# technosaurus/PDMP3

Hardware: AMD Instinct MI355X
Metric: MP3 frames/sec (44.1 kHz stereo 320 kbps), transforms-only hot path (higher is better)
Workload: dtype f32; 1 GPU; C2 (BASELINE configs[1]): 2048 stereo frames = 4096 granules per GPU per step, pre-Huffman-decoded spectra resident in HBM, one stream; frames_per_gpu=2048, granules_per_gpu=4096, seed=0x5eed0000c2, chunk_frames=auto

## Files before the change

pdmp3_amd/csrc/decode_core.h:

```cpp
#pragma once

#include <math.h>
#include <stdint.h>
#include <string.h>
#include "../../include/pdmp3_hip.h"

namespace pdmp3 {
struct ConstBank;
}

#if defined(__HIPCC__)
#define PD_FN __device__ __forceinline__
#define PD_SLOW_FN __device__ __attribute__((noinline))
#define PD_MFN __device__ __forceinline__
#define PD_HD __host__ __device__ __forceinline__
#define PD_FMA(a, b, c) __builtin_fmaf((a), (b), (c))
#define PD_CLOCK() __builtin_amdgcn_s_memtime()
#define PD_UNROLL _Pragma("unroll")
#define PD_UNROLL_N(n) _Pragma(PD_STR_(unroll n))
#define PD_STR_(x) #x
#define PD_NOUNROLL _Pragma("nounroll")
#define PD_SCHED_FENCE() __builtin_amdgcn_sched_barrier(0)
#define PD_PIN(x) asm volatile("" : "+v"(x))
#define PD_ANY(c) (__builtin_amdgcn_ballot_w64(c) != 0ull)
#define PD_LANE() ((int)(threadIdx.x & 63))
#define PD_UNIFORM(x) __builtin_amdgcn_readfirstlane((int)(x))
#define PD_SHFL_XOR(v, m) __shfl_xor((v), (m))
#define PD_WAVE_SYNC()                                       \
  __builtin_amdgcn_fence(__ATOMIC_RELEASE, "wavefront");    \
  __builtin_amdgcn_wave_barrier();                          \
  __builtin_amdgcn_fence(__ATOMIC_ACQUIRE, "wavefront")
#define PD_STORE_DEVICE(p, v) __hip_atomic_store((p), (v), __ATOMIC_RELAXED, __HIP_MEMORY_SCOPE_AGENT)
#define PD_LOAD_DEVICE(p) __hip_atomic_load((p), __ATOMIC_RELAXED, __HIP_MEMORY_SCOPE_AGENT)
#define PD_VMEM_DRAIN() asm volatile("s_waitcnt vmcnt(0)" ::: "memory")
#define PD_SLEEP() __builtin_amdgcn_s_sleep(4)
#define PD_SETPRIO(x) __builtin_amdgcn_s_setprio(x)
#define PD_LDS_FLAG(p) (*(volatile __attribute__((address_space(3))) unsigned*)(p))
#define PD_BALLOT(c) ((unsigned long long)__builtin_amdgcn_ballot_w64(c))
namespace pdmp3 {
typedef const __attribute__((address_space(4))) ConstBank* BankPtr;
}
#define PD_LAUNDER(p) asm volatile("" : "+s"(p))
#define PD_UNIFORM_PTR(T, p) ((T)(((unsigned long long)(unsigned)PD_UNIFORM((int)((unsigned long long)(p) >> 32)) << 32) | (unsigned)PD_UNIFORM((int)(unsigned long long)(p))))
#define PD_UNCHECKED_INDEX(v, lo, n) (v)
#define PD_FMED3(x, lo, hi) __builtin_amdgcn_fmed3f((x), (lo), (hi))
namespace pdmp3 {
typedef float f32x2 __attribute__((ext_vector_type(2)));
typedef unsigned short u16x2 __attribute__((ext_vector_type(2)));
typedef float f32x4 __attribute__((ext_vector_type(4)));
__device__ __forceinline__ f32x2 fma2(f32x2 a, f32x2 b, f32x2 c) { return __builtin_elementwise_fma(a, b, c); }
__device__ __forceinline__ f32x4 mfma16(float a, float b, f32x4 c) { return __builtin_amdgcn_mfma_f32_16x16x4f32(a, b, c, 0, 0, 0); }
__device__ __forceinline__ void permlane32_swap(int& a, int& b) {
  const auto r = __builtin_amdgcn_permlane32_swap((unsigned)a, (unsigned)b, false, false);
  a = (int)r[0];
  b = (int)r[1];
}
__device__ __forceinline__ void mul9_rtz_32767(const float* x, float* p) {
#define PD_M(n, m) "v_mul_f32 %" #n ", 0x46fffe00, %" #m "\n\t"
  asm volatile(
      "s_setreg_imm32_b32 hwreg(HW_REG_MODE, 0, 2), 3\n\t"
      "s_nop 1\n\t"
      PD_M(0, 9) PD_M(1, 10) PD_M(2, 11) PD_M(3, 12) PD_M(4, 13) PD_M(5, 14) PD_M(6, 15) PD_M(7, 16) PD_M(8, 17)
      "s_setreg_imm32_b32 hwreg(HW_REG_MODE, 0, 2), 0\n\t"
      "s_nop 1"
      : "=&v"(p[0]), "=&v"(p[1]), "=&v"(p[2]), "=&v"(p[3]), "=&v"(p[4]), "=&v"(p[5]), "=&v"(p[6]), "=&v"(p[7]), "=&v"(p[8])
      : "v"(x[0]), "v"(x[1]), "v"(x[2]), "v"(x[3]), "v"(x[4]), "v"(x[5]), "v"(x[6]), "v"(x[7]), "v"(x[8]));
#undef PD_M
}
__device__ __forceinline__ void mul18_rtz_32767(const float* x, float* p) {
  mul9_rtz_32767(x, p);
  mul9_rtz_32767(x + 9, p + 9);
}
}
#else
namespace pdmp3 {
namespace emu {
int lane();
void wave_sync();
void wave_yield();
float shfl_xor(float v, int mask);
bool any(bool c);
unsigned long long ballot(bool c);
void mfma16(float a, float b, float* cd);
void permlane32_swap(int* a, int* b);
}
}
#define PD_FN static inline
#define PD_SLOW_FN static
#define PD_MFN inline
#define PD_HD static inline
#define PD_FMA(a, b, c) __builtin_fmaf((a), (b), (c))
#define PD_CLOCK() 0ull
#define PD_UNROLL
#define PD_UNROLL_N(n)
#define PD_NOUNROLL
#define PD_SCHED_FENCE() ((void)0)
#define PD_PIN(x) ((void)0)
#define PD_ANY(c) (::pdmp3::emu::any(c))
#define PD_LANE() (::pdmp3::emu::lane())
#define PD_UNIFORM(x) ((int)(x))
#define PD_SHFL_XOR(v, m) (::pdmp3::emu::shfl_xor((v), (m)))
#define PD_WAVE_SYNC() ::pdmp3::emu::wave_sync()
#define PD_STORE_DEVICE(p, v) (*(p) = (v))
#define PD_LOAD_DEVICE(p) (*(p))
#define PD_VMEM_DRAIN() ::pdmp3::emu::wave_sync()
#define PD_SLEEP() ::pdmp3::emu::wave_yield()
#define PD_SETPRIO(x) ((void)0)
#define PD_LDS_FLAG(p) (*(volatile unsigned*)(p))
#define PD_BALLOT(c) (::pdmp3::emu::ballot(c))
namespace pdmp3 {
typedef const ConstBank* BankPtr;
}
#define PD_LAUNDER(p) ((void)0)
#define PD_UNIFORM_PTR(T, p) (p)
#define PD_UNCHECKED_INDEX(v, lo, n) ((unsigned)((v) - (lo)) < (unsigned)(n) ? (v) : 0)
namespace pdmp3 {
typedef float f32x2 __attribute__((vector_size(8)));
typedef unsigned short u16x2 __attribute__((vector_size(4)));
typedef float f32x4 __attribute__((vector_size(16)));
static inline f32x2 fma2(f32x2 a, f32x2 b, f32x2 c) { return (f32x2){__builtin_fmaf(a[0], b[0], c[0]), __builtin_fmaf(a[1], b[1], c[1])}; }
static inline f32x4 mfma16(float a, float b, f32x4 c) {
  float cd[4] = {c[0], c[1], c[2], c[3]};
  emu::mfma16(a, b, cd);
  return (f32x4){cd[0], cd[1], cd[2], cd[3]};
}
static inline void permlane32_swap(int& a, int& b) { emu::permlane32_swap(&a, &b); }
static inline float pd_fmed3_host(float x, float lo, float hi) {
  if (x != x) return lo < hi ? lo : hi;
  return x < lo ? lo : (x > hi ? hi : x);
}
static inline void mul18_rtz_32767(const float* x, float* p) {
  for (int t = 0; t < 18; t++) {
    const double d = (double)x[t] * 32767.0;
    float f = (float)d;
    if (f == f && !__builtin_isinf(f) && __builtin_fabs((double)f) > __builtin_fabs(d)) f = __builtin_nextafterf(f, 0.0f);
    else if (__builtin_isinf(f) && !__builtin_isinf(x[t])) f = __builtin_copysignf(0x1.fffffep+127f, f);
    p[t] = f;
  }
}
}
#define PD_FMED3(x, lo, hi) (::pdmp3::pd_fmed3_host((x), (lo), (hi)))
#endif

#ifndef PD_EXP_SKIP
#define PD_EXP_SKIP 0
#endif
#ifndef PD_C36_MQ
#define PD_C36_MQ 1
#endif
#ifndef PD_CHUNK_FAST_REQUANT
#define PD_CHUNK_FAST_REQUANT 0
#endif
#ifndef PD_PRIO_MFMA
#define PD_PRIO_MFMA 2
#endif
#ifndef PD_PRIO_WINDOW
#define PD_PRIO_WINDOW 0
#endif
#ifndef PD_PRIO_REQUANT
#define PD_PRIO_REQUANT 1
#endif
// ... 99 lines not shown
  int nch, sfreq, mode, mode_ext;
  int ver;
  int lsf_scale;
  int iso;
  int count1_0, count1_1, flags0, flags1;
  PD_MFN int flags(int ch) const { return ch ? flags1 : flags0; }
  PD_MFN bool is_short(int ch) const {
    const int f = flags(ch);
    return (f & PDMP3_GC_WIN_SWITCH) && ((f & PDMP3_GC_BLOCK_TYPE_MASK) >> PDMP3_GC_BLOCK_TYPE_SHIFT) == 2;
  }
  PD_MFN bool is_mixed(int ch) const { return (flags(ch) & PDMP3_GC_MIXED) != 0; }
  PD_MFN int block_type(int ch) const { return (flags(ch) & PDMP3_GC_BLOCK_TYPE_MASK) >> PDMP3_GC_BLOCK_TYPE_SHIFT; }
  PD_MFN int kind(int ch) const { return is_short(ch) ? (is_mixed(ch) ? 2 : 1) : 0; }
};

template <bool RARE = true>
PD_FN GranuleInfo granule_info(const WaveData& L) {
  GranuleInfo g;
  const uint32_t w0 = (uint32_t)PD_UNIFORM(*reinterpret_cast<const uint32_t*>(&L.side[0][0]));
  const uint32_t w1 = (uint32_t)PD_UNIFORM(*reinterpret_cast<const uint32_t*>(&L.side[1][0]));
  const int fr = PD_UNIFORM(L.side[0][7]);
  g.fr = fr;
  g.iso = PD_UNIFORM(L.side[0][offsetof(pdmp3_gc_side, iso)]);
  g.sfreq = fr & PDMP3_FR_SFREQ_MASK;
  if (g.sfreq > 2) g.sfreq = 2;
  g.ver = 0;
  g.lsf_scale = 0;
  if (RARE) {
    const int lsf0 = PD_UNIFORM(L.side[0][offsetof(pdmp3_gc_side, lsf)]);
    g.ver = lsf0 & PDMP3_LSF_VERSION_MASK;
    if (g.ver > 2) g.ver = 2;
  }
  if (RARE && g.ver) {
    g.sfreq += 3 * g.ver;
    g.iso |= PDMP3_GC_ISO_MS_ALL | PDMP3_GC_ISO_IS_SHORT | PDMP3_GC_ISO_IS_STD;
    g.lsf_scale = (PD_UNIFORM(L.side[1][offsetof(pdmp3_gc_side, lsf)]) & PDMP3_LSF_IS_SCALE) ? 1 : 0;
  }
  g.mode = (fr & PDMP3_FR_MODE_MASK) >> PDMP3_FR_MODE_SHIFT;
  g.mode_ext = (fr & PDMP3_FR_MODEEXT_MASK) >> PDMP3_FR_MODEEXT_SHIFT;
  g.nch = (g.mode == 3) ? 1 : 2;
  g.count1_0 = (int)(w0 & 0xffffu);
  g.count1_1 = (int)(w1 & 0xffffu);
  g.flags0 = (int)(w0 >> 24);
  g.flags1 = (int)(w1 >> 24);
  return g;
}

PD_FN bool frame_is_rare(const pdmp3_gc_side* rec) {
  const uint8_t* b = reinterpret_cast<const uint8_t*>(rec);
  const unsigned fr = b[7];
  const bool is = ((fr & PDMP3_FR_MODE_MASK) >> PDMP3_FR_MODE_SHIFT) == 1 && (fr & (1u << PDMP3_FR_MODEEXT_SHIFT));
  return is || (b[offsetof(pdmp3_gc_side, lsf)] & PDMP3_LSF_VERSION_MASK) != 0;
}

PD_HD uint32_t f2u(float f) { uint32_t u; memcpy(&u, &f, 4); return u; }
PD_HD float u2f(uint32_t u) { float f; memcpy(&f, &u, 4); return f; }


PD_FN void state_zero(int lane, LaneRegs& R) {
  (void)lane;
  for (int m = 0; m < kOvlRegs; m++) R.ovl[m] = 0.0f;
  for (int s = 0; s < kHistSlots; s++) { R.he[s] = 0.0f; R.ho[s] = 0.0f; }
}

template <bool TAPS = true>
PD_FN void lane_init(int lane, WaveData& L, LaneRegs& R, BankPtr cb, const GlobalTables& T) {
  const int i = lane & 31;
  (void)cb;
  R.idx_e = (i < 16) ? 16 + i : ((i == 16) ? 0 : 48 - i);
  R.idx_o = (i <= 16) ? 16 - i : i - 16;
  if (TAPS) {
    for (int k = 0; k < 8; k++) {
      R.we[k] = T.taps[k * 64 + lane];
      R.wo[k] = T.taps[(8 + k) * 64 + lane];
    }
  }
  state_zero(lane, R);
  if (lane < 4) L.peek[lane] = 1.0f;
  for (int k = 0; k < 10; k++) R.bi[k] = T.frag_long[k * 64 + lane];
  for (int k = 0; k < 8; k++) R.bm[k] = T.frag_mat[k * 64 + lane];
}

PD_HD int fast_line(int lane, int i) { return i < 4 ? 2 * lane + 128 * i : 512 + lane; }
PD_FN unsigned band_addr_of(const GlobalTables& T, int sfreq, int line) {
  return (unsigned)((T.linetab[(size_t)sfreq * 3 * 576 + line] >> 10) << 2);
}

PD_FN void tab_load_image(int tid, int nthr, TabLds& S, const GlobalTables& T, int sfreq) {
  const Chunk16* src = reinterpret_cast<const Chunk16*>(reinterpret_cast<const char*>(T.tab_image) + (size_t)sfreq * sizeof(TabLds));
  Chunk16* dst = reinterpret_cast<Chunk16*>(&S);
  for (int k = tid; k < (int)(sizeof(TabLds) / 16); k += nthr) dst[k] = src[k];
}
PD_FN void load_linetab(int lane, TabLds& S, const GlobalTables& T, int sfreq) { tab_load_image(lane, 64, S, T, sfreq); }

constexpr int kStateFloats = 64 * (kOvlRegs + 2 * kHistSlots);

PD_FN void state_load(int lane, LaneRegs& R, const float* st) {
  for (int m = 0; m < kOvlRegs; m++) R.ovl[m] = st[m * 64 + lane];
  for (int s = 0; s < kHistSlots; s++) {
    R.he[s] = st[(kOvlRegs + s) * 64 + lane];
    R.ho[s] = st[(kOvlRegs + kHistSlots + s) * 64 + lane];
  }
}

PD_FN void state_load_ch1(int lane, LaneRegs& R, const float* st) {
  for (int m = 8; m < 16; m++) R.ovl[m] = st[m * 64 + lane];
  if (lane >= 32) {
    R.ovl[16] = st[16 * 64 + lane];
    R.ovl[17] = st[17 * 64 + lane];
    for (int s = 0; s < kHistSlots; s++) {
      R.he[s] = st[(kOvlRegs + s) * 64 + lane];
      R.ho[s] = st[(kOvlRegs + kHistSlots + s) * 64 + lane];
    }
  }
}

PD_FN void state_store(int lane, const LaneRegs& R, float* st) {
  for (int m = 0; m < kOvlRegs; m++) st[m * 64 + lane] = R.ovl[m];
  for (int s = 0; s < kHistSlots; s++) {
    st[(kOvlRegs + s) * 64 + lane] = R.he[s];
    st[(kOvlRegs + kHistSlots + s) * 64 + lane] = R.ho[s];
  }
}

PD_FN void ph_prefetch(int lane, LaneRegs& R, const int16_t* spectra_g, const pdmp3_gc_side* side_g) {
  const Chunk16* src = reinterpret_cast<const Chunk16*>(spectra_g);
  R.pf0 = src[lane];
  R.pf1 = src[lane + 64];
  if (lane < 16) {
    R.pf2 = src[lane + 128];
    R.pf3 = reinterpret_cast<const Chunk16*>(side_g)[lane];
  }
}

PD_FN void ph_commit(int lane, WaveData& L, const LaneRegs& R) {
  Chunk16* dst = reinterpret_cast<Chunk16*>(&L.spec[0][0]);
  dst[lane] = R.pf0;
  dst[lane + 64] = R.pf1;
  if (lane < 16) {
    dst[lane + 128] = R.pf2;
    reinterpret_cast<Chunk16*>(&L.side[0][0])[lane] = R.pf3;
  }
}

PD_HD float pow2_quarter(int k) {
  const int j = k & 3;
// ... 994 lines not shown
    if (g + 1 >= gp.g_end) return;
    const int nx = gran_next_place(gp);
    const unsigned tag = gran_tag(gp, g + 1);
    GranMb& mb = gp.mb[nx];
    gran_lds_wait_tag(&mb.free, tag);
    float* tb = gran_tails_box(gp.wl[nx]);
    float* rb = gran_rows_box(gp.wl[nx]);
    for (int m = 0; m < kOvlRegs; m++) tb[m * 64 + lane] = R.ovl[m];
    for (int s = 0; s < kHistSlots; s++) {
      if (i < 16) rb[s * 64 + ch * 32 + 16 + i] = R.he[s];
      if (i <= 16) rb[s * 64 + ch * 32 + 16 - i] = R.ho[s];
    }
    PD_WAVE_SYNC();
    if (lane == 0) { PD_LDS_FLAG(&mb.tails_full) = tag; PD_LDS_FLAG(&mb.rows_full) = tag; }
    return;
  }
  const bool far = gp.w == gp.wpw - 1;
  float* tails = far ? a.chain_state + (size_t)g * kGranFloats : nullptr;
  if (far) {
    for (int m = 0; m < kOvlRegs; m++) PD_STORE_DEVICE(&tails[m * 64 + lane], R.ovl[m]);
    float* rows = tails + kOvlRegs * 64;
    for (int s = 0; s < kHistSlots; s++) {
      if (i < 16) PD_STORE_DEVICE(&rows[s * 64 + ch * 32 + 16 + i], R.he[s]);
      if (i <= 16) PD_STORE_DEVICE(&rows[s * 64 + ch * 32 + 16 - i], R.ho[s]);
    }
    PD_VMEM_DRAIN();
    if (lane == 0) { PD_STORE_DEVICE(a.chain_flag + 2 * (size_t)g, a.chain_epoch); PD_STORE_DEVICE(a.chain_flag + 2 * (size_t)g + 1, a.chain_epoch); }
  } else {
    GranMb& mb = gp.mb[gp.w + 1];
    gran_lds_wait(&mb.free);
    float* tb = gran_tails_box(gp.wl[gp.w + 1]);
    float* rb = gran_rows_box(gp.wl[gp.w + 1]);
    for (int m = 0; m < kOvlRegs; m++) tb[m * 64 + lane] = R.ovl[m];
    for (int s = 0; s < kHistSlots; s++) {
      if (i < 16) rb[s * 64 + ch * 32 + 16 + i] = R.he[s];
      if (i <= 16) rb[s * 64 + ch * 32 + 16 - i] = R.ho[s];
    }
    PD_WAVE_SYNC();
    if (lane == 0) { PD_LDS_FLAG(&mb.tails_full) = 1u; PD_LDS_FLAG(&mb.rows_full) = 1u; }
  }
}
constexpr int kGranFarPolls = 1 << 13;
PD_FN bool gran_far_wait(const DecodeArgs& a, int g, int k, bool bounded) {
  if (bounded && (a.debug_flags & PD_DEBUG_FAR_TIMEOUT)) return false;
  for (int n = 0; (unsigned)PD_UNIFORM(PD_LOAD_DEVICE(a.chain_flag + 2 * (size_t)(g - 1) + k)) != a.chain_epoch; ++n) {
    if (bounded && n >= kGranFarPolls) return false;
    PD_SLEEP();
  }
  asm volatile("" ::: "memory");
  return true;
}

PD_FN void ph_imdct(int lane, const WaveData& L, const TabLds& S, const LaneRegs& R, BankPtr cb, const GlobalTables& T, float* y1, float* y2,
                    const GranuleInfo* gi = nullptr) {
  const GranuleInfo g = gi ? *gi : granule_info(L);
  const int j = lane & 15, kq = lane >> 4;
  const bool any_short = g.is_short(0) || g.is_short(1);
  {
    const int cl = lane >> 5, sb = lane & 31;
    const bool lwsf = (g.flags(cl) & PDMP3_GC_WIN_SWITCH) != 0;
    const bool llow = lwsf && g.is_mixed(cl) && sb < 2;
    const bool lshort = g.is_short(cl) && !llow;
    const float* x = &L.xr[cl][18 * sb];
    float in[18];
    PD_UNROLL for (int m = 0; m < 18; m++) in[m] = x[m];
    float y[4] = {0.0f, 0.0f, 0.0f, 0.0f};
    PD_UNROLL for (int m = 0; m < 18; m++)
      PD_UNROLL for (int q = 0; q < 4; q++) y[q] = PD_FMA(in[m], PD_C36(cb, c36x, q, m), y[q]);
    const float* w = S.win[llow ? 0 : g.block_type(cl)];
    y[0] = y[0] * w[16]; y[1] = y[1] * w[17]; y[2] = y[2] * w[34]; y[3] = y[3] * w[35];
    if (any_short) {
      float ys[4] = {0.0f, 0.0f, 0.0f, 0.0f};
      PD_UNROLL for (int m = 0; m < 18; m++)
        PD_UNROLL for (int q = 0; q < 4; q++) ys[q] = PD_FMA(in[m], PD_C36(cb, s36x, q, m), ys[q]);
      PD_UNROLL for (int q = 0; q < 4; q++) y[q] = lshort ? ys[q] : y[q];
    }
    y1[16] = y[0]; y1[17] = y[1]; y2[16] = y[2]; y2[17] = y[3];
  }
  PD_UNROLL for (int cc = 0; cc < 2; cc++) {
    const int ch = 1 - cc;
    const bool shrt = g.is_short(ch);
    const bool wsf = (g.flags(ch) & PDMP3_GC_WIN_SWITCH) != 0;
    const bool mixrows = wsf && g.is_mixed(ch);
    const int bt = g.block_type(ch);
    float bfr[10];
    if (shrt) {
        PD_UNROLL for (int k = 0; k < 10; k++) bfr[k] = T.frag_short[k * 64 + lane];
        PD_UNROLL for (int k = 0; k < 10; k++) PD_PIN(bfr[k]);
      }
    else { PD_UNROLL for (int k = 0; k < 10; k++) bfr[k] = R.bi[k]; }
    f32x4 acc[2][2];
    float afr[2][5];
    PD_UNROLL for (int h = 0; h < 2; h++)
      PD_UNROLL for (int kk = 0; kk < 5; kk++) {
        const int k = 4 * kk + kq;
        afr[h][kk] = L.xr[ch][18 * (h ? 31 - j : j) + (k < 18 ? k : 0)];
        if (k >= 18) afr[h][kk] = 0.0f;
      }
    PD_UNROLL for (int h = 0; h < 2; h++)
      PD_UNROLL for (int nt = 0; nt < 2; nt++) acc[h][nt] = mfma16(afr[h][0], bfr[nt], (f32x4){0, 0, 0, 0});
    PD_UNROLL for (int kk = 1; kk < 5; kk++)
      PD_UNROLL for (int h = 0; h < 2; h++)
        PD_UNROLL for (int nt = 0; nt < 2; nt++) acc[h][nt] = mfma16(afr[h][kk], bfr[kk * 2 + nt], acc[h][nt]);
    f32x4 accl[2];
    PD_UNROLL for (int nt = 0; nt < 2; nt++) accl[nt] = acc[0][nt];
    if (shrt && mixrows) {
      PD_UNROLL for (int nt = 0; nt < 2; nt++) accl[nt] = mfma16(afr[0][0], R.bi[nt], (f32x4){0, 0, 0, 0});
      PD_UNROLL for (int kk = 1; kk < 5; kk++)
        PD_UNROLL for (int nt = 0; nt < 2; nt++) accl[nt] = mfma16(afr[0][kk], R.bi[kk * 2 + nt], accl[nt]);
    }
    const float* wb = S.win[bt];
    const float* w0 = S.win[0];
    const float wb1 = wb[j], wb2 = wb[18 + j];
    const float w01 = w0[j], w02 = w0[18 + j];
    PD_UNROLL for (int h = 0; h < 2; h++)
      PD_UNROLL for (int r = 0; r < 4; r++) {
        const bool lowrow = mixrows && h == 0 && kq == 0 && r < 2;
        float a1 = acc[h][0][r], a2 = acc[h][1][r];
        if (h == 0 && lowrow) { a1 = accl[0][r]; a2 = accl[1][r]; }
        const bool win_folded = shrt && !lowrow;
        const float f1 = lowrow ? w01 : wb1, f2 = lowrow ? w02 : wb2;
        if (!win_folded) { a1 = a1 * f1; a2 = a2 * f2; }
        y1[ch * 8 + h * 4 + r] = a1;
        y2[ch * 8 + h * 4 + r] = a2;
      }
  }
}
PD_FN void ph_overlap_matrix(int lane, WaveData& L, const LaneRegs& R, const float* y1, const float* ovl) {
  const int j = lane & 15, kq = lane >> 4;
  {
    const int cl = lane >> 5, sb = lane & 31;
    const float o16 = y1[16] + ovl[16];
    float o17 = y1[17] + ovl[17];
    if (sb & 1) o17 = -o17;
    const float p16 = PD_SHFL_XOR(o16, 31), p17 = PD_SHFL_XOR(o17, 31);
    if (sb < 16) {
      L.lo[0][2 * cl + 0][sb] = o16 + p16; L.lo[1][2 * cl + 0][sb] = o16 - p16;
      L.lo[0][2 * cl + 1][sb] = o17 + p17; L.lo[1][2 * cl + 1][sb] = o17 - p17;
    }
// ... 28 lines not shown
      const float a = (j < 4) ? L.lo[0][j & 3][4 * kq + r] : 0.0f;
      const float b = (j < 4) ? L.lo[1][j & 3][4 * kq + r] : 0.0f;
      me = mfma16(a, R.bm[r], me);
      mo = mfma16(b, R.bm[4 + r], mo);
    }
    if (kq == 0) {
      PD_UNROLL for (int r = 0; r < 4; r++) {
        const int ch = r >> 1, t = 16 + (r & 1);
        L.hyb[ch][t][2 * j] = me[r]; L.hyb[ch][t][2 * j + 1] = mo[r];
      }
    }
  }
}
PD_FN void ph_window_own(int lane, const WaveData& L, const TabLds& S, LaneRegs& R, float* acc) {
  const int ch = lane >> 5;
  PD_UNROLL for (int k = 0; k < 8; k++) { R.we[k] = S.taps[k][lane & 31]; R.wo[k] = S.taps[8 + k][lane & 31]; }
  float E[18], O[18];
  PD_UNROLL for (int t = 0; t < 18; t++) { E[t] = L.hyb[ch][t][R.idx_e]; O[t] = L.hyb[ch][t][R.idx_o]; }
  PD_UNROLL for (int t = 0; t < 18; t++) {
    float s = 0.0f;
    PD_UNROLL for (int k = 0; k < 8; k++) {
      if (t - 2 * k >= 0) s = PD_FMA(R.we[k], E[t - 2 * k], s);
      if (t - 2 * k - 1 >= 0) s = PD_FMA(R.wo[k], O[t - 2 * k - 1], s);
    }
    acc[t] = s;
  }
}
template <bool F32>
PD_FN void ph_window_hist(int lane, WaveData& L, const LaneRegs& R, const float* acc, int16_t* pcm_g, float* pcmf_g) {
  float sum[18];
  PD_UNROLL for (int t = 0; t < 18; t++) {
    float s = acc[t];
    PD_UNROLL for (int k = 0; k < 8; k++) {
      if (t - 2 * k < 0) s = PD_FMA(R.we[k], R.he[kHistSlots + t - 2 * k], s);
      if (t - 2 * k - 1 < 0) s = PD_FMA(R.wo[k], R.ho[kHistSlots + t - 2 * k - 1], s);
    }
    sum[t] = s;
  }
  pcm_emit<F32, true>(lane, L, 2, true, sum, pcm_g, pcmf_g);
}

template <bool F32>
PD_SLOW_FN void gran_slow_chunk(DecodeArgs a, GlobalTables T, BankPtr cb, int f, WaveData* L, TabLds* S, GranPos second, bool publish,
                                LaneRegs* state_only) {
  cb = PD_UNIFORM_PTR(BankPtr, cb);
  f = PD_UNIFORM(f);
  gran_tabs_wait(second);
  run_chunk<false, false, F32, false>(a, T, cb, f, *L, *S, publish ? &second : nullptr, state_only);
}

template <bool F32, bool RING = false>
PD_FN void run_granule(const DecodeArgs& a, const GlobalTables& T, BankPtr cb, int g, WaveData& L, TabLds& S, const GranPos& gp,
                       bool fresh, bool h5, bool next_takes, const LaneRegs& pf, LaneRegs* Rp = nullptr, bool emit = true,
                       bool zero_in = false, bool halo_in = false, int g_pf = -1) {
  LaneRegs R;
  (void)Rp;
  int lane_ = PD_LANE();
  if (RING) PD_PIN(lane_);
  const int lane = lane_;
  const int f = g >> 1, gr = g & 1;
  const bool from_caller = fresh && gr == 0 && f == 0 && a.state_in && !(reinterpret_cast<const uint8_t*>(a.side)[7] & PDMP3_FR_RESET);
  const bool from_zero = (fresh && gr == 0 && !from_caller) || (RING && zero_in);
  const bool from_chain = !from_caller && !from_zero;
  const unsigned tag = gran_tag(gp, g);
#define PD_GT(k) if (a.prof) { const unsigned long long t_ = PD_CLOCK(); if (lane == 0) a.prof[(size_t)g * kProfSlots + (k)] = t_; }
  PD_GT(1)
  R.pf0 = pf.pf0; R.pf1 = pf.pf1; R.pf2 = pf.pf2; R.pf3 = pf.pf3;
  const bool far_sender = !RING && gp.w == gp.wpw - 1 && next_takes;
  if (far_sender) PD_SETPRIO(2);
  PD_PHASE(lane_init<false>(lane, L, R, cb, T))
  if (h5 && (gr == 1 || !fresh)) {
    if (!RING) PD_SETPRIO(3);
    float pk = 0.0f;
    gran_tabs_wait(gp);
    if (gr == 0) {
      LaneRegs R1;
      R1.ovl[0] = 0.0f;
      PD_PHASE(ph_prefetch(lane, R1, a.spectra + (size_t)(g - 1) * 1152, a.side + (size_t)(g - 1) * 2))
      PD_PHASE(ph_commit(lane, L, R1))
      PD_PHASE(ph_scales(lane, L))
      PD_PHASE((ph_requant<false, 1, false, true, false, false>(lane, L, S, cb, T, nullptr, nullptr)))
      PD_PHASE(ph_antialias(lane, L, cb, true))
      PD_PHASE(ph_peek_tail(lane, L, S, R1, T))
      GranMb& mb = gp.mb[gran_next_place(gp)];
      if (lane < 3) mb.peek_tail[lane] = R1.ovl[0];
      PD_WAVE_SYNC();
      if (RING) gran_lds_flag_tag(lane, &mb.peek_full, gran_tag(gp, g + 1));
      else gran_lds_flag(lane, &mb.peek_full);
    } else {
      LaneRegs R0;
      float tail = 0.0f;
      PD_PHASE(ph_prefetch(lane, R0, a.spectra + (size_t)(g - 1) * 1152, a.side + (size_t)(g - 1) * 2))
      if (fresh && f == 0 && a.state_in && !(reinterpret_cast<const uint8_t*>(a.side)[7] & PDMP3_FR_RESET) && lane < 3) tail = a.state_in[lane];
      PD_PHASE(ph_commit(lane, L, R0))
      PD_PHASE(ph_scales(lane, L))
      PD_PHASE((ph_requant<false, 1, false, true, false, false>(lane, L, S, cb, T, nullptr, nullptr)))
      PD_PHASE(ph_antialias(lane, L, cb, true))
      const float head = ph_peek_head(lane, L, S, T);
      PD_WAVE_SYNC();
      if (!fresh) {
        if (RING) gran_lds_wait_tag(&gp.mb[gp.w].peek_full, tag);
        else gran_lds_wait(&gp.mb[gp.w].peek_full);
        tail = lane < 3 ? gp.mb[gp.w].peek_tail[lane] : 0.0f;
      }
      pk = head + tail;
    }
    PD_PHASE(ph_commit(lane, L, R))
    if (gr == 1) { PD_PHASE(if (lane < 3) L.peek[lane] = pk) }
  } else {
    PD_PHASE(ph_commit(lane, L, R))
  }
  PD_GT(2)
  gran_tabs_wait(gp);
  PD_LAUNDER(cb);
  const GranuleInfo gi = granule_info<false>(L);
  if (!(PD_EXP_SKIP & 1)) { PD_PHASE((ph_requant<false, 9, true, true, true, false>(lane, L, S, cb, T, nullptr, nullptr, &gi))) }
  PD_GT(3)
  if (!RING && !(h5 && (gr == 1 || !fresh))) {
    const int q = gp.w >> 2;
    if (q == 1) PD_SETPRIO(1); else if (q == 2) PD_SETPRIO(2); else if (q == 3) PD_SETPRIO(3); else PD_SETPRIO(0);
  }
  if (!(PD_EXP_SKIP & 2)) { PD_PHASE(ph_antialias(lane, L, cb, false, &gi)) }
  float y1[kOvlRegs], y2[kOvlRegs];
  if (PD_EXP_SKIP & 4) { PD_UNROLL for (int m = 0; m < kOvlRegs; m++) { y1[m] = L.xr[0][m * 64 + lane]; y2[m] = L.xr[1][m * 64 + lane]; } }
  else { PD_PHASE(ph_imdct(lane, L, S, R, cb, T, y1, y2, &gi)) }
  PD_GT(4)
  if (RING) gran_lds_flag_tag(lane, &gp.mb[gp.w].free, tag);
  else if (gp.w > 0) gran_lds_flag(lane, &gp.mb[gp.w].free);
  if (next_takes) {
    if (RING) { PD_PHASE(gran_send_tails_ring(lane, y2, g, gp)) }
    else { PD_PHASE(gran_send_tails(lane, y2, a, g, gp)) }
  }
  PD_GT(5)
  float ovl[kOvlRegs];
  bool have_halo = false;
  LaneRegs H;
  if (from_caller) { PD_UNROLL for (int m = 0; m < kOvlRegs; m++) ovl[m] = a.state_in[m * 64 + lane]; }
  else if (from_zero) { PD_UNROLL for (int m = 0; m < kOvlRegs; m++) ovl[m] = 0.0f; }
  else if (RING ? !halo_in : gp.w > 0) {
    if (RING) gran_lds_wait_tag(&gp.mb[gp.w].tails_full, tag);
    else gran_lds_wait(&gp.mb[gp.w].tails_full);
    const float* box = gran_tails_box(L);
    PD_UNROLL for (int m = 0; m < kOvlRegs; m++) ovl[m] = box[m * 64 + lane];
    PD_WAVE_SYNC();
  } else if (!RING && gran_far_wait(a, g, 0, true)) {
    const float* st = a.chain_state + (size_t)(g - 1) * kGranFloats;
    PD_UNROLL for (int m = 0; m < kOvlRegs; m++) ovl[m] = PD_LOAD_DEVICE(&st[m * 64 + lane]);
  } else {
    PD_WAVE_SYNC();
    gran_slow_chunk<F32>(a, T, cb, f, &L, &S, gp, false, &H);
    PD_WAVE_SYNC();
    PD_UNROLL for (int m = 0; m < kOvlRegs; m++) ovl[m] = H.ovl[m];
    have_halo = true;
  }
  PD_GT(6)
  if (PD_EXP_SKIP & 8) { L.hyb[0][lane & 15][lane >> 2] = y1[0] + ovl[1]; } else { PD_PHASE(ph_overlap_matrix(lane, L, R, y1, ovl)) }
  PD_GT(7)
  if (g == 2 * a.n_frames - 1 && a.state_out) {
    float* so = a.state_out;
    const int ch = lane >> 5;
    PD_UNROLL for (int m = 0; m < kOvlRegs; m++) so[m * 64 + lane] = y2[m];
    PD_UNROLL for (int s = 0; s < kHistSlots; s++) {
      so[(kOvlRegs + s) * 64 + lane] = L.hyb[ch][3 + s][R.idx_e];
      so[(kOvlRegs + kHistSlots + s) * 64 + lane] = L.hyb[ch][3 + s][R.idx_o];
    }
  }
  if (next_takes) {
    if (RING) { PD_PHASE(gran_send_rows_ring(lane, L, g, gp)) }
    else { PD_PHASE(gran_send_rows(lane, L, a, g, gp)) }
  }
  if (far_sender && !(gr == 1 && h5)) PD_SETPRIO(0);
  PD_GT(8)
  (void)g_pf;
  if (RING && !emit) {
    if (from_chain) gran_lds_wait_tag(&gp.mb[gp.w].rows_full, tag);
    PD_GT(11)
    return;
  }
  float acc[18];
  if (PD_EXP_SKIP & 16) { PD_UNROLL for (int t = 0; t < 18; t++) acc[t] = L.hyb[0][t][lane & 31]; } else { PD_PHASE(ph_window_own(lane, L, S, R, acc)) }
  PD_GT(9)
  if (have_halo) { PD_UNROLL for (int s = 0; s < kHistSlots; s++) { R.he[s] = H.he[s]; R.ho[s] = H.ho[s]; } }
  else if (from_caller) {
    PD_UNROLL for (int s = 0; s < kHistSlots; s++) {
      R.he[s] = a.state_in[(kOvlRegs + s) * 64 + lane];
      R.ho[s] = a.state_in[(kOvlRegs + kHistSlots + s) * 64 + lane];
    }
  } else if (from_zero) { PD_UNROLL for (int s = 0; s < kHistSlots; s++) { R.he[s] = 0.0f; R.ho[s] = 0.0f; } }
  else if (RING || gp.w > 0) {
    if (RING) gran_lds_wait_tag(&gp.mb[gp.w].rows_full, tag);
    else gran_lds_wait(&gp.mb[gp.w].rows_full);
    const float* rows = gran_rows_box(L) + (lane >> 5) * 32;
    PD_UNROLL for (int s = 0; s < kHistSlots; s++) { R.he[s] = rows[s * 64 + R.idx_e]; R.ho[s] = rows[s * 64 + R.idx_o]; }
  } else {
    gran_far_wait(a, g, 1, false);
    const float* rows = a.chain_state + (size_t)(g - 1) * kGranFloats + kOvlRegs * 64 + (lane >> 5) * 32;
    PD_UNROLL for (int s = 0; s < kHistSlots; s++) { R.he[s] = PD_LOAD_DEVICE(&rows[s * 64 + R.idx_e]); R.ho[s] = PD_LOAD_DEVICE(&rows[s * 64 + R.idx_o]); }
  }
  (void)from_chain;
  PD_GT(10)
  if (PD_EXP_SKIP & 32) { a.pcm[(size_t)f * 2304 + gr * 1152 + lane] = (int16_t)(acc[0] + acc[17] + R.he[0] + R.ho[14]); } else { PD_PHASE(ph_window_hist<F32>(lane, L, R, acc, a.pcm + (size_t)f * 2304 + gr * 1152, F32 ? a.pcm_f32 + (size_t)f * 2304 + gr * 1152 : nullptr)) }
  PD_GT(11)
#undef PD_GT
}

template <bool F32, bool RING = false>
PD_FN void run_granule_wave(const DecodeArgs& a, const GlobalTables& T, BankPtr cb, int g, WaveData& L, TabLds& S, const GranPos& gp,
                            const LaneRegs& pf, LaneRegs* Rp = nullptr, int g_emit = 0, bool halo_by_wave = false, int g_pf = -1) {
  const int f = g >> 1, gr = g & 1;
  const uint8_t fb = reinterpret_cast<const uint8_t*>(a.side + (size_t)f * 4)[7];
  const uint8_t pb = reinterpret_cast<const uint8_t*>(a.side + (size_t)(f > 0 ? f - 1 : 0) * 4)[7];
  const uint8_t nb = reinterpret_cast<const uint8_t*>(a.side + (size_t)(f + 1 < a.n_frames ? f + 1 : f) * 4)[7];
  const uint8_t fl = reinterpret_cast<const uint8_t*>(a.side + (size_t)(2 * f + 1) * 2 + 1)[3];
  const bool rare = frame_is_rare(a.side + (size_t)f * 4);
  const bool prev_rare = frame_is_rare(a.side + (size_t)(f > 0 ? f - 1 : 0) * 4);
  const bool next_rare = frame_is_rare(a.side + (size_t)(f + 1 < a.n_frames ? f + 1 : f) * 4);
  const bool stereo = ((fb & PDMP3_FR_MODE_MASK) >> PDMP3_FR_MODE_SHIFT) != 3 && !rare;
  const bool fresh = f == 0 || (fb & PDMP3_FR_RESET);
  const bool prev_stereo = ((pb & PDMP3_FR_MODE_MASK) >> PDMP3_FR_MODE_SHIFT) != 3 && !prev_rare;
  const bool chained = stereo && (fresh || prev_stereo);
  const bool h5 = (fl & PDMP3_GC_WIN_SWITCH) && ((fl & PDMP3_GC_BLOCK_TYPE_MASK) >> PDMP3_GC_BLOCK_TYPE_SHIFT) == 2;
  bool next_takes = false;
  if (chained) {
    next_takes = gr == 0 || (f + 1 < a.n_frames && ((nb & PDMP3_FR_MODE_MASK) >> PDMP3_FR_MODE_SHIFT) != 3 && !(nb & PDMP3_FR_RESET) && !next_rare);
    if (RING) {
      if (g + 1 >= gp.g_end) next_takes = false;
      const bool halo_frame = g < g_emit;
      run_granule<F32, true>(a, T, cb, g, L, S, gp, fresh, h5, next_takes, pf, Rp, !halo_frame, halo_frame && gr == 0 && !fresh,
                             halo_by_wave && g == g_emit && !fresh, g_pf);
    } else run_granule<F32, false>(a, T, cb, g, L, S, gp, fresh, h5, next_takes, pf);
    return;
  }
  if (gr == 0) {
    GranPos second = gp;
    second.w = gp.w + 1;
    if (RING) {
      gran_slow_chunk<F32>(a, T, cb, f, &L, &S, second, true, nullptr);
    } else gran_slow_chunk<F32>(a, T, cb, f, &L, &S, second, true, nullptr);
  }
}

template <bool F32>
PD_FN void run_granule_ring(const DecodeArgs& a, const GlobalTables& T, BankPtr cb, WaveData& L, TabLds& S, GranPos gp, int f0, int f1) {
  const int lane = PD_LANE();
  int g_emit = 2 * f0;
  bool halo_by_wave = false;
  gp.ring = 1;
  gp.g_base = g_emit;
  gp.g_end = 2 * f1;
  if (f0 > 0) {
    const uint8_t b0 = reinterpret_cast<const uint8_t*>(a.side + (size_t)f0 * 4)[7];
    const uint8_t b1 = reinterpret_cast<const uint8_t*>(a.side + (size_t)(f0 - 1) * 4)[7];
    const uint8_t b2 = reinterpret_cast<const uint8_t*>(a.side + (size_t)(f0 > 1 ? f0 - 2 : 0) * 4)[7];
    const bool st0 = ((b0 & PDMP3_FR_MODE_MASK) >> PDMP3_FR_MODE_SHIFT) != 3 && !frame_is_rare(a.side + (size_t)f0 * 4);
    const bool st1 = ((b1 & PDMP3_FR_MODE_MASK) >> PDMP3_FR_MODE_SHIFT) != 3 && !frame_is_rare(a.side + (size_t)(f0 - 1) * 4);
    const bool st2 = ((b2 & PDMP3_FR_MODE_MASK) >> PDMP3_FR_MODE_SHIFT) != 3 && !frame_is_rare(a.side + (size_t)(f0 > 1 ? f0 - 2 : 0) * 4);
    const bool needs_state = st0 && !(b0 & PDMP3_FR_RESET) && st1;
    if (needs_state) {
      const bool prev_goes_granule_way = (b1 & PDMP3_FR_RESET) || f0 == 1 || st2;
      if (prev_goes_granule_way) gp.g_base = g_emit - 2;
      else halo_by_wave = true;
    }
  }
  GlobalTables Tl = T;
  for (int g = gp.g_base + gp.w; g < gp.g_end; g += gp.wpw) {
    PD_LAUNDER(Tl.taps); PD_LAUNDER(Tl.frag_long); PD_LAUNDER(Tl.frag_mat);
    if (a.prof) { const unsigned long long t_ = PD_CLOCK(); if (lane == 0) a.prof[(size_t)g * kProfSlots] = t_; }
    LaneRegs pf;
    ph_prefetch(lane, pf, a.spectra + (size_t)g * 1152, a.side + (size_t)g * 2);
    run_granule_wave<F32, true>(a, Tl, cb, g, L, S, gp, pf, nullptr, g_emit, halo_by_wave, -1);
    PD_WAVE_SYNC();
  }
}

}
```

pdmp3_amd/csrc/engine.hip:

```cpp
#include <hip/hip_runtime.h>

#include <stddef.h>
#include <stdio.h>
#include <stdlib.h>
#include <string.h>

#include "decode_core.h"
#include "engine_internal.h"
#include "gen_core.h"
#include "host_tables.h"
#include "unpack_core.h"
#include <new>

using namespace pdmp3;

#ifndef PDMP3_WAVES_PER_EU
#define PDMP3_WAVES_PER_EU 2
#endif

__constant__ ConstBank c_bank;

__device__ __forceinline__ int xcd_contiguous(int b, int n) {
  const int q = n >> 3, r = n & 7, x = b & 7;
  return (x < r ? x * (q + 1) : r * (q + 1) + (x - r) * q) + (b >> 3);
}

template <bool DUMP, bool F32 = false, int WPW = 1>
__global__ __launch_bounds__(64 * WPW, PDMP3_WAVES_PER_EU) void k_decode(DecodeArgs a, GlobalTables T, int n_chunks, unsigned* rare_flag, unsigned rare_epoch) {
  __shared__ WaveLds L[WPW];
  const int w = threadIdx.x >> 6;
  const int n_wgs = (n_chunks + WPW - 1) / WPW;
  const int chunk = xcd_contiguous((int)blockIdx.x, n_wgs) * WPW + w;
  if (chunk >= n_chunks) return;
  if (DUMP) { run_chunk<DUMP, false, F32, true, true>(a, T, (BankPtr)&c_bank, chunk, L[w], L[w].tab); return; }
  if (rare_flag && chunk_is_rare(a, chunk)) {
    if ((threadIdx.x & 63) == 0) __hip_atomic_store(rare_flag, rare_epoch, __ATOMIC_RELAXED, __HIP_MEMORY_SCOPE_AGENT);
    return;
  }
  run_chunk<DUMP, false, F32, true, false>(a, T, (BankPtr)&c_bank, chunk, L[w], L[w].tab);
}

template <bool F32>
__global__ __launch_bounds__(64, PDMP3_WAVES_PER_EU) void k_decode_rare(DecodeArgs a, GlobalTables T, int n_chunks, int always, const unsigned* rare_flag, unsigned rare_epoch) {
  __shared__ WaveLds L[1];
  const int chunk = (int)blockIdx.x;
  if (chunk >= n_chunks) return;
  if (!always) {
    if (__hip_atomic_load(rare_flag, __ATOMIC_RELAXED, __HIP_MEMORY_SCOPE_AGENT) != rare_epoch) return;
    if (!chunk_is_rare(a, chunk)) return;
  }
  run_chunk<false, false, F32, true, true>(a, T, (BankPtr)&c_bank, chunk, L[0], L[0].tab);
}

template <bool F32, int W>
__global__ __launch_bounds__(64 * W) __attribute__((amdgpu_waves_per_eu(W / 4, W / 4))) void k_decode_g(DecodeArgs a, GlobalTables T) {
  __shared__ WaveData L[W];
  __shared__ TabLds S;
  __shared__ GranMb mb[W];
  __shared__ unsigned tabs_ready;
  static_assert(sizeof(WaveData) * W + sizeof(TabLds) + sizeof(GranMb) * W + 16 <= 160 * 1024, "one workgroup of 16 waves per CU");
  const int tid = (int)threadIdx.x;
  const unsigned long long t_entry = a.prof ? PD_CLOCK() : 0ull;
  const int w = tid >> 6;
  const int g = (int)blockIdx.x * W + w;
  const bool valid = g < 2 * a.n_frames;
  LaneRegs pf;
  if (valid) ph_prefetch(tid & 63, pf, a.spectra + (size_t)g * 1152, a.side + (size_t)g * 2);
  if (tid < W * (int)(sizeof(GranMb) / 4)) reinterpret_cast<unsigned*>(mb)[tid] = 0u;
  if (tid == 0) tabs_ready = 0u;
  __syncthreads();
  tab_load_image(tid, 64 * W, S, T, a.sf_hint);
  __builtin_amdgcn_fence(__ATOMIC_RELEASE, "wavefront");
  __builtin_amdgcn_wave_barrier();
  if ((tid & 63) == 0) atomicAdd(&tabs_ready, 1u);
  if (!valid) return;
  if (a.prof && (tid & 63) == 0) a.prof[(size_t)g * kProfSlots] = t_entry;
  const GranPos gp{L, mb, w, W, &tabs_ready};
  run_granule_wave<F32>(a, T, (BankPtr)&c_bank, g, L[w], S, gp, pf);
}

#if defined(PDMP3_WITH_RING_KERNEL)
template <bool F32>
__global__ __launch_bounds__(64 * 16) __attribute__((amdgpu_waves_per_eu(4, 4))) void k_decode_p(DecodeArgs a, GlobalTables T, int frames_per_wg) {
  constexpr int W = 16;
  __shared__ WaveData L[W];
  __shared__ TabLds S;
  __shared__ GranMb mb[W];
  __shared__ unsigned tabs_ready;
  const int tid = (int)threadIdx.x;
  const int w = tid >> 6;
  if (tid < W * (int)(sizeof(GranMb) / 4)) reinterpret_cast<unsigned*>(mb)[tid] = 0u;
  if (tid == 0) tabs_ready = 0u;
  __syncthreads();
  tab_load_image(tid, 64 * W, S, T, a.sf_hint);
  __builtin_amdgcn_fence(__ATOMIC_RELEASE, "wavefront");
  __builtin_amdgcn_wave_barrier();
  if ((tid & 63) == 0) atomicAdd(&tabs_ready, 1u);
  const int f0 = (int)blockIdx.x * frames_per_wg;
  int f1 = f0 + frames_per_wg;
  if (f1 > a.n_frames) f1 = a.n_frames;
  const GranPos gp{L, mb, w, W, &tabs_ready, 1, 2 * f0, 2 * f1};
  run_granule_ring<F32>(a, T, (BankPtr)&c_bank, L[w], S, gp, f0, f1);
}
#endif

__global__ __launch_bounds__(64, PDMP3_WAVES_PER_EU) void k_decode_prof(DecodeArgs a, GlobalTables T) {
  __shared__ WaveLds L[1];
  const int w = threadIdx.x >> 6;
  run_chunk<false, true, false, true, false>(a, T, (BankPtr)&c_bank, (int)blockIdx.x, L[w], L[w].tab);
}

__global__ __launch_bounds__(256) void k_lsf_pair(const int16_t* in_sp, const pdmp3_gc_side* in_sd, int n_frames, int16_t* out_sp, pdmp3_gc_side* out_sd) {
  const int p = blockIdx.x;
  const uint4 zero = make_uint4(0, 0, 0, 0);
  for (int gr = 0; gr < 2; gr++) {
    const int f = 2 * p + gr;
    const uint4* ssp = reinterpret_cast<const uint4*>(in_sp + (size_t)f * 2304);
    const uint4* ssd = reinterpret_cast<const uint4*>(in_sd + (size_t)f * 4);
    uint4* dsp = reinterpret_cast<uint4*>(out_sp + (size_t)p * 2304 + gr * 1152);
    uint4* dsd = reinterpret_cast<uint4*>(out_sd + (size_t)p * 4 + gr * 2);
    for (int k = threadIdx.x; k < 144 + 16; k += blockDim.x) {
      if (k < 144) dsp[k] = f < n_frames ? ssp[k] : zero;
      else dsd[k - 144] = f < n_frames ? ssd[k - 144] : zero;
    }
  }
}

__global__ __launch_bounds__(64) void k_generate(uint64_t seed, int64_t first, int16_t* spectra, pdmp3_gc_side* side) {
  const int64_t gc = blockIdx.x;
  const int64_t f = gc >> 2;
  gen_gc(seed, first + f, (unsigned)((gc >> 1) & 1), (unsigned)(gc & 1), (int)threadIdx.x,
// ... 572 lines not shown
```

Measured before the change: 111.8 million frames/s.

## Hoist table, side-info and short-block fragment loads ahead of the barrier

The granule kernel now issues its global loads for the LDS table image, the short-window MFMA fragments and the per-frame side-info dwords before the initial __syncthreads, holding them in registers and writing them to LDS afterward. Short-block IMDCT fragments are read from LDS instead of global memory, and routing decisions use the preloaded dwords instead of scattered byte loads. The goal is to overlap load latency with setup and cut dependent global round-trips. The cost is more live registers across the barrier and extra LDS use, which could lower occupancy or cause spills.

```diff
diff --git a/pdmp3_amd/csrc/decode_core.h b/pdmp3_amd/csrc/decode_core.h
--- a/pdmp3_amd/csrc/decode_core.h
+++ b/pdmp3_amd/csrc/decode_core.h
@@ -36,6 +36,7 @@
 #define PD_SLEEP() __builtin_amdgcn_s_sleep(4)
 #define PD_SETPRIO(x) __builtin_amdgcn_s_setprio(x)
 #define PD_LDS_FLAG(p) (*(volatile __attribute__((address_space(3))) unsigned*)(p))
+#define PD_LDS_F32(p) ((const __attribute__((address_space(3))) float*)(p))
 #define PD_BALLOT(c) ((unsigned long long)__builtin_amdgcn_ballot_w64(c))
 namespace pdmp3 {
 typedef const __attribute__((address_space(4))) ConstBank* BankPtr;
@@ -107,6 +108,7 @@
 #define PD_SLEEP() ::pdmp3::emu::wave_yield()
 #define PD_SETPRIO(x) ((void)0)
 #define PD_LDS_FLAG(p) (*(volatile unsigned*)(p))
+#define PD_LDS_F32(p) (p)
 #define PD_BALLOT(c) (::pdmp3::emu::ballot(c))
 namespace pdmp3 {
 typedef const ConstBank* BankPtr;
@@ -312,6 +314,33 @@
   const bool is = ((fr & PDMP3_FR_MODE_MASK) >> PDMP3_FR_MODE_SHIFT) == 1 && (fr & (1u << PDMP3_FR_MODEEXT_SHIFT));
   return is || (b[offsetof(pdmp3_gc_side, lsf)] & PDMP3_LSF_VERSION_MASK) != 0;
 }
+constexpr int kGcFrameDw = (int)(offsetof(pdmp3_gc_side, frame) / 4), kGcFrameSh = 8 * (int)(offsetof(pdmp3_gc_side, frame) % 4);
+constexpr int kGcLsfDw = (int)(offsetof(pdmp3_gc_side, lsf) / 4), kGcLsfSh = 8 * (int)(offsetof(pdmp3_gc_side, lsf) % 4);
+constexpr int kGcFlagsSh = 8 * (int)offsetof(pdmp3_gc_side, flags);
+static_assert(offsetof(pdmp3_gc_side, flags) < 4 && sizeof(pdmp3_gc_side) == 128, "GranRoute reads whole dwords of the records");
+PD_HD unsigned frame_byte_dw(uint32_t frame_dw) { return (frame_dw >> kGcFrameSh) & 0xffu; }
+PD_HD bool frame_is_rare_dw(uint32_t frame_dw, uint32_t lsf_dw) {
+  const unsigned fr = frame_byte_dw(frame_dw);
+  const bool is = ((fr & PDMP3_FR_MODE_MASK) >> PDMP3_FR_MODE_SHIFT) == 1 && (fr & (1u << PDMP3_FR_MODEEXT_SHIFT));
+  return is | (((lsf_dw >> kGcLsfSh) & PDMP3_LSF_VERSION_MASK) != 0);
+}
+
+struct GranRoute {
+  uint32_t fr_p, fr_f, fr_n;
+  uint32_t lsf_p, lsf_f, lsf_n;
+  uint32_t fl;
+};
+PD_FN void gran_route_load(GranRoute& rt, const pdmp3_gc_side* side, int n_frames, int f) {
+  constexpr int kRecDw = (int)(sizeof(pdmp3_gc_side) / 4);
+  const uint32_t* s = reinterpret_cast<const uint32_t*>(side);
+  const uint32_t* sf = s + (size_t)f * 4 * kRecDw;
+  const uint32_t* sp = s + (size_t)(f > 0 ? f - 1 : 0) * 4 * kRecDw;
+  const uint32_t* sn = s + (size_t)(f + 1 < n_frames ? f + 1 : f) * 4 * kRecDw;
+  rt.fr_f = sf[kGcFrameDw]; rt.lsf_f = sf[kGcLsfDw];
+  rt.fr_p = sp[kGcFrameDw]; rt.lsf_p = sp[kGcLsfDw];
+  rt.fr_n = sn[kGcFrameDw]; rt.lsf_n = sn[kGcLsfDw];
+  rt.fl = sf[3 * kRecDw];
+}
 
 PD_HD uint32_t f2u(float f) { uint32_t u; memcpy(&u, &f, 4); return u; }
 PD_HD float u2f(uint32_t u) { float f; memcpy(&f, &u, 4); return f; }
@@ -352,6 +381,30 @@
   for (int k = tid; k < (int)(sizeof(TabLds) / 16); k += nthr) dst[k] = src[k];
 }
 PD_FN void load_linetab(int lane, TabLds& S, const GlobalTables& T, int sfreq) { tab_load_image(lane, 64, S, T, sfreq); }
+
+constexpr int kTabImageChunks = (int)(sizeof(TabLds) / 16);
+constexpr int kFragShortFloats = 10 * 64;
+constexpr int kFragShortChunks = kFragShortFloats * 4 / 16;
+template <int NTHR>
+struct TabFetch { Chunk16 c[(kTabImageChunks + kFragShortChunks + NTHR - 1) / NTHR]; };
+template <int NTHR>
+PD_FN void tab_fetch_issue(int tid, TabFetch<NTHR>& F, const GlobalTables& T, int sfreq) {
+  const Chunk16* img = reinterpret_cast<const Chunk16*>(reinterpret_cast<const char*>(T.tab_image) + (size_t)sfreq * sizeof(TabLds));
+  const Chunk16* fs = reinterpret_cast<const Chunk16*>(T.frag_short);
+  PD_UNROLL for (int i = 0; i < (int)(sizeof(F.c) / sizeof(F.c[0])); i++) {
+    const int k = tid + i * NTHR;
+    const Chunk16* p = k < kTabImageChunks ? img + k : fs + (k - kTabImageChunks);
+    if (k < kTabImageChunks + kFragShortChunks) F.c[i] = *p;
+  }
+}
+template <int NTHR>
+PD_FN void tab_fetch_store(int tid, const TabFetch<NTHR>& F, TabLds& S, float* frag_short_lds) {
+  PD_UNROLL for (int i = 0; i < (int)(sizeof(F.c) / sizeof(F.c[0])); i++) {
+    const int k = tid + i * NTHR;
+    if (k < kTabImageChunks) reinterpret_cast<Chunk16*>(&S)[k] = F.c[i];
+    else if (k < kTabImageChunks + kFragShortChunks) reinterpret_cast<Chunk16*>(frag_short_lds)[k - kTabImageChunks] = F.c[i];
+  }
+}
 
 constexpr int kStateFloats = 64 * (kOvlRegs + 2 * kHistSlots);
 
@@ -1452,10 +1505,14 @@
 }
 
 PD_FN void ph_imdct(int lane, const WaveData& L, const TabLds& S, const LaneRegs& R, BankPtr cb, const GlobalTables& T, float* y1, float* y2,
-                    const GranuleInfo* gi = nullptr) {
+                    const GranuleInfo* gi = nullptr, const float* frag_short_lds = nullptr) {
   const GranuleInfo g = gi ? *gi : granule_info(L);
   const int j = lane & 15, kq = lane >> 4;
   const bool any_short = g.is_short(0) || g.is_short(1);
+  float bsh[10];
+  if (frag_short_lds && any_short) {
+    PD_UNROLL for (int k = 0; k < 10; k++) bsh[k] = PD_LDS_F32(frag_short_lds)[k * 64 + lane];
+  }
   {
     const int cl = lane >> 5, sb = lane & 31;
     const bool lwsf = (g.flags(cl) & PDMP3_GC_WIN_SWITCH) != 0;
@@ -1484,7 +1541,8 @@
     const bool mixrows = wsf && g.is_mixed(ch);
     const int bt = g.block_type(ch);
     float bfr[10];
-    if (shrt) {
+    if (shrt && frag_short_lds) { PD_UNROLL for (int k = 0; k < 10; k++) bfr[k] = bsh[k]; }
+    else if (shrt) {
         PD_UNROLL for (int k = 0; k < 10; k++) bfr[k] = T.frag_short[k * 64 + lane];
         PD_UNROLL for (int k = 0; k < 10; k++) PD_PIN(bfr[k]);
       }
@@ -1619,14 +1677,16 @@
 template <bool F32, bool RING = false>
 PD_FN void run_granule(const DecodeArgs& a, const GlobalTables& T, BankPtr cb, int g, WaveData& L, TabLds& S, const GranPos& gp,
                        bool fresh, bool h5, bool next_takes, const LaneRegs& pf, LaneRegs* Rp = nullptr, bool emit = true,
-                       bool zero_in = false, bool halo_in = false, int g_pf = -1) {
+                       bool zero_in = false, bool halo_in = false, int g_pf = -1, int fr_own = -1,
+                       const float* frag_short_lds = nullptr) {
   LaneRegs R;
   (void)Rp;
   int lane_ = PD_LANE();
   if (RING) PD_PIN(lane_);
   const int lane = lane_;
   const int f = g >> 1, gr = g & 1;
-  const bool from_caller = fresh && gr == 0 && f == 0 && a.state_in && !(reinterpret_cast<const uint8_t*>(a.side)[7] & PDMP3_FR_RESET);
+#define PD_FRAME0_BYTE() (fr_own >= 0 ? (unsigned)fr_own : (unsigned)reinterpret_cast<const uint8_t*>(a.side)[7])
+  const bool from_caller = fresh && gr == 0 && f == 0 && a.state_in && !(PD_FRAME0_BYTE() & PDMP3_FR_RESET);
   const bool from_zero = (fresh && gr == 0 && !from_caller) || (RING && zero_in);
   const bool from_chain = !from_caller && !from_zero;
   const unsigned tag = gran_tag(gp, g);
@@ -1658,7 +1718,7 @@
       LaneRegs R0;
       float tail = 0.0f;
       PD_PHASE(ph_prefetch(lane, R0, a.spectra + (size_t)(g - 1) * 1152, a.side + (size_t)(g - 1) * 2))
-      if (fresh && f == 0 && a.state_in && !(reinterpret_cast<const uint8_t*>(a.side)[7] & PDMP3_FR_RESET) && lane < 3) tail = a.state_in[lane];
+      if (fresh && f == 0 && a.state_in && !(PD_FRAME0_BYTE() & PDMP3_FR_RESET) && lane < 3) tail = a.state_in[lane];
       PD_PHASE(ph_commit(lane, L, R0))
       PD_PHASE(ph_scales(lane, L))
       PD_PHASE((ph_requant<false, 1, false, true, false, false>(lane, L, S, cb, T, nullptr, nullptr)))
@@ -1690,7 +1750,7 @@
   if (!(PD_EXP_SKIP & 2)) { PD_PHASE(ph_antialias(lane, L, cb, false, &gi)) }
   float y1[kOvlRegs], y2[kOvlRegs];
   if (PD_EXP_SKIP & 4) { PD_UNROLL for (int m = 0; m < kOvlRegs; m++) { y1[m] = L.xr[0][m * 64 + lane]; y2[m] = L.xr[1][m * 64 + lane]; } }
-  else { PD_PHASE(ph_imdct(lane, L, S, R, cb, T, y1, y2, &gi)) }
+  else { PD_PHASE(ph_imdct(lane, L, S, R, cb, T, y1, y2, &gi, frag_short_lds)) }
   PD_GT(4)
   if (RING) gran_lds_flag_tag(lane, &gp.mb[gp.w].free, tag);
   else if (gp.w > 0) gran_lds_flag(lane, &gp.mb[gp.w].free);
@@ -1769,19 +1829,19 @@
   if (PD_EXP_SKIP & 32) { a.pcm[(size_t)f * 2304 + gr * 1152 + lane] = (int16_t)(acc[0] + acc[17] + R.he[0] + R.ho[14]); } else { PD_PHASE(ph_window_hist<F32>(lane, L, R, acc, a.pcm + (size_t)f * 2304 + gr * 1152, F32 ? a.pcm_f32 + (size_t)f * 2304 + gr * 1152 : nullptr)) }
   PD_GT(11)
 #undef PD_GT
+#undef PD_FRAME0_BYTE
 }
 
 template <bool F32, bool RING = false>
 PD_FN void run_granule_wave(const DecodeArgs& a, const GlobalTables& T, BankPtr cb, int g, WaveData& L, TabLds& S, const GranPos& gp,
-                            const LaneRegs& pf, LaneRegs* Rp = nullptr, int g_emit = 0, bool halo_by_wave = false, int g_pf = -1) {
+                            const LaneRegs& pf, const GranRoute& rt, LaneRegs* Rp = nullptr, int g_emit = 0, bool halo_by_wave = false,
+                            int g_pf = -1, const float* frag_short_lds = nullptr) {
   const int f = g >> 1, gr = g & 1;
-  const uint8_t fb = reinterpret_cast<const uint8_t*>(a.side + (size_t)f * 4)[7];
-  const uint8_t pb = reinterpret_cast<const uint8_t*>(a.side + (size_t)(f > 0 ? f - 1 : 0) * 4)[7];
-  const uint8_t nb = reinterpret_cast<const uint8_t*>(a.side + (size_t)(f + 1 < a.n_frames ? f + 1 : f) * 4)[7];
-  const uint8_t fl = reinterpret_cast<const uint8_t*>(a.side + (size_t)(2 * f + 1) * 2 + 1)[3];
-  const bool rare = frame_is_rare(a.side + (size_t)f * 4);
-  const bool prev_rare = frame_is_rare(a.side + (size_t)(f > 0 ? f - 1 : 0) * 4);
-  const bool next_rare = frame_is_rare(a.side + (size_t)(f + 1 < a.n_frames ? f + 1 : f) * 4);
+  const unsigned fb = frame_byte_dw(rt.fr_f), pb = frame_byte_dw(rt.fr_p), nb = frame_byte_dw(rt.fr_n);
+  const unsigned fl = (rt.fl >> kGcFlagsSh) & 0xffu;
+  const bool rare = frame_is_rare_dw(rt.fr_f, rt.lsf_f);
+  const bool prev_rare = frame_is_rare_dw(rt.fr_p, rt.lsf_p);
+  const bool next_rare = frame_is_rare_dw(rt.fr_n, rt.lsf_n);
   const bool stereo = ((fb & PDMP3_FR_MODE_MASK) >> PDMP3_FR_MODE_SHIFT) != 3 && !rare;
   const bool fresh = f == 0 || (fb & PDMP3_FR_RESET);
   const bool prev_stereo = ((pb & PDMP3_FR_MODE_MASK) >> PDMP3_FR_MODE_SHIFT) != 3 && !prev_rare;
@@ -1794,8 +1854,8 @@
       if (g + 1 >= gp.g_end) next_takes = false;
       const bool halo_frame = g < g_emit;
       run_granule<F32, true>(a, T, cb, g, L, S, gp, fresh, h5, next_takes, pf, Rp, !halo_frame, halo_frame && gr == 0 && !fresh,
-                             halo_by_wave && g == g_emit && !fresh, g_pf);
-    } else run_granule<F32, false>(a, T, cb, g, L, S, gp, fresh, h5, next_takes, pf);
+                             halo_by_wave && g == g_emit && !fresh, g_pf, (int)fb, frag_short_lds);
+    } else run_granule<F32, false>(a, T, cb, g, L, S, gp, fresh, h5, next_takes, pf, nullptr, true, false, false, -1, (int)fb, frag_short_lds);
     return;
   }
   if (gr == 0) {
@@ -1805,6 +1865,13 @@
       gran_slow_chunk<F32>(a, T, cb, f, &L, &S, second, true, nullptr);
     } else gran_slow_chunk<F32>(a, T, cb, f, &L, &S, second, true, nullptr);
   }
+}
+template <bool F32, bool RING = false>
+PD_FN void run_granule_wave(const DecodeArgs& a, const GlobalTables& T, BankPtr cb, int g, WaveData& L, TabLds& S, const GranPos& gp,
+                            const LaneRegs& pf, LaneRegs* Rp = nullptr, int g_emit = 0, bool halo_by_wave = false, int g_pf = -1) {
+  GranRoute rt;
+  gran_route_load(rt, a.side, a.n_frames, g >> 1);
+  run_granule_wave<F32, RING>(a, T, cb, g, L, S, gp, pf, rt, Rp, g_emit, halo_by_wave, g_pf);
 }
 
 template <bool F32>
diff --git a/pdmp3_amd/csrc/engine.hip b/pdmp3_amd/csrc/engine.hip
--- a/pdmp3_amd/csrc/engine.hip
+++ b/pdmp3_amd/csrc/engine.hip
@@ -58,25 +58,32 @@
   __shared__ TabLds S;
   __shared__ GranMb mb[W];
   __shared__ unsigned tabs_ready;
-  static_assert(sizeof(WaveData) * W + sizeof(TabLds) + sizeof(GranMb) * W + 16 <= 160 * 1024, "one workgroup of 16 waves per CU");
+  __shared__ alignas(16) float frag_short_lds[kFragShortFloats];
+  static_assert(sizeof(WaveData) * W + sizeof(TabLds) + sizeof(GranMb) * W + 16 + sizeof(float) * kFragShortFloats <= 160 * 1024,
+                "one workgroup of 16 waves per CU");
   const int tid = (int)threadIdx.x;
   const unsigned long long t_entry = a.prof ? PD_CLOCK() : 0ull;
   const int w = tid >> 6;
   const int g = (int)blockIdx.x * W + w;
   const bool valid = g < 2 * a.n_frames;
+  const int gl = valid ? g : 2 * a.n_frames - 1;
+  TabFetch<64 * W> tf;
+  tab_fetch_issue<64 * W>(tid, tf, T, a.sf_hint);
   LaneRegs pf;
-  if (valid) ph_prefetch(tid & 63, pf, a.spectra + (size_t)g * 1152, a.side + (size_t)g * 2);
+  ph_prefetch(tid & 63, pf, a.spectra + (size_t)gl * 1152, a.side + (size_t)gl * 2);
+  GranRoute rt;
+  gran_route_load(rt, a.side, a.n_frames, gl >> 1);
   if (tid < W * (int)(sizeof(GranMb) / 4)) reinterpret_cast<unsigned*>(mb)[tid] = 0u;
   if (tid == 0) tabs_ready = 0u;
   __syncthreads();
-  tab_load_image(tid, 64 * W, S, T, a.sf_hint);
+  tab_fetch_store<64 * W>(tid, tf, S, frag_short_lds);
   __builtin_amdgcn_fence(__ATOMIC_RELEASE, "wavefront");
   __builtin_amdgcn_wave_barrier();
   if ((tid & 63) == 0) atomicAdd(&tabs_ready, 1u);
   if (!valid) return;
   if (a.prof && (tid & 63) == 0) a.prof[(size_t)g * kProfSlots] = t_entry;
   const GranPos gp{L, mb, w, W, &tabs_ready};
-  run_granule_wave<F32>(a, T, (BankPtr)&c_bank, g, L[w], S, gp, pf);
+  run_granule_wave<F32>(a, T, (BankPtr)&c_bank, g, L[w], S, gp, pf, rt, nullptr, 0, false, -1, frag_short_lds);
 }
 
 #if defined(PDMP3_WITH_RING_KERNEL)
```

After: 111.7 million frames/s. About the same (-0.1%).
